# speechbrain/speechbrain

Hardware: NVIDIA H100
Metric: audio-sec/sec (RTFx) Conformer-L ASR, batch=32x10s@16kHz (higher is better)
Workload: dtype fp16 operands, fp32 accumulate/residual/softmax

## Files before the change

speechbrain_b200/csrc/encoder_ops.cu:

```cuda
#include <algorithm>

#include "common.cuh"
#include "sbk_internal.h"

namespace sbk {

constexpr int LN_MAX_PER_LANE = 32;

template <bool OUT_HALF, bool PDL, bool DUAL = false>
__global__ void __launch_bounds__(256)
layernorm_rows_kernel(const float* __restrict__ x, void* __restrict__ out, const float* __restrict__ gamma,
                      const float* __restrict__ beta, int M, int D, float eps, int act_silu,
                      __half* __restrict__ out2 = nullptr, const float* __restrict__ gamma2 = nullptr,
                      const float* __restrict__ beta2 = nullptr) {
    const int row = blockIdx.x * (blockDim.x >> 5) + (threadIdx.x >> 5);
    const int lane = threadIdx.x & 31;
    const int nv = D >> 2;
    float4 gp[PDL ? LN_MAX_PER_LANE / 4 : 1], bp[PDL ? LN_MAX_PER_LANE / 4 : 1];
    if constexpr (PDL) {
#pragma unroll
        for (int i = 0; i < LN_MAX_PER_LANE / 4; ++i) {
            const int vi = lane + i * 32;
            if (vi < nv && row < M) {
                gp[i] = __ldg(reinterpret_cast<const float4*>(gamma + vi * 4));
// ... 365 lines not shown
    const int ch = blockIdx.x * blockDim.x + threadIdx.x, b = blockIdx.y;
    if (ch >= D) return;
    float* cb = carry + static_cast<size_t>(b) * halo * D + ch;
    for (int j = 0; j < halo; ++j) {
        const int src = j + n - halo;
        cb[static_cast<size_t>(j) * D] = src >= 0 ? glu[(static_cast<size_t>(b) * n + src) * D + ch]
                                                  : (has_old ? cb[static_cast<size_t>(j + n) * D] : 0.0f);
    }
}

int dwconv_carry(const float* glu, int B, int n, int D, int K, bool has_old, float* carry, cudaStream_t stream) {
    const int halo = (K - 1) / 2;
    if (halo == 0) return SBK_OK;
    dwconv_carry_kernel<<<dim3(ceil_div(D, 128), B), 128, 0, stream>>>(glu, n, D, halo, has_old ? 1 : 0, carry);
    SBK_LAUNCH_CHECK();
    return SBK_OK;
}

void dwconv_repack_taps(const float* src, int D, int K, float* dst) {
    for (int ch = 0; ch < D; ++ch)
        for (int k = 0; k < K; ++k) dst[static_cast<size_t>(k) * D + ch] = src[static_cast<size_t>(ch) * K + k];
}

constexpr int CSGU_KMAX = CSGU_TAP_ROWS, CSGU_HALO = (CSGU_KMAX - 1) / 2;
constexpr int CSGU_TT = 64, CSGU_CC = 64, CSGU_THREADS = 256;
constexpr int CSGU_FPT = CSGU_TT / (CSGU_THREADS / CSGU_CC);
constexpr int CSGU_ROWS = CSGU_TT + CSGU_KMAX - 1;

__global__ void __launch_bounds__(256)
csgu_stats_kernel(const __half* __restrict__ u, int M, int C, float eps, float2* __restrict__ stats) {
    const int row = blockIdx.x * (blockDim.x >> 5) + (threadIdx.x >> 5);
    if (row >= M) return;
    const int lane = threadIdx.x & 31, C2 = C >> 1, nv = C2 >> 3;
    const uint4* src = reinterpret_cast<const uint4*>(u + static_cast<size_t>(row) * C + C2);
    float s = 0.0f;
    for (int j = lane; j < nv; j += 32) {
        const uint4 w = __ldg(src + j);
        const __half2* h = reinterpret_cast<const __half2*>(&w);
#pragma unroll
        for (int q = 0; q < 4; ++q) { const float2 f = __half22float2(h[q]); s += f.x + f.y; }
    }
    const float mean = warp_sum(s) / C2;
    float v = 0.0f;
    for (int j = lane; j < nv; j += 32) {
        const uint4 w = __ldg(src + j);
        const __half2* h = reinterpret_cast<const __half2*>(&w);
#pragma unroll
        for (int q = 0; q < 4; ++q) {
            const float2 f = __half22float2(h[q]);
            v += (f.x - mean) * (f.x - mean) + (f.y - mean) * (f.y - mean);
        }
    }
    const float rstd = rsqrtf(warp_sum(v) / C2 + eps);
    if (lane == 0) stats[row] = make_float2(mean, rstd);
}

__global__ void __launch_bounds__(CSGU_THREADS)
csgu_conv_gate_kernel(const __half* __restrict__ u, int T, int C, const float2* __restrict__ stats,
                      const float* __restrict__ gamma, const float* __restrict__ beta, const float* __restrict__ taps,
                      const float* __restrict__ bias, __half* __restrict__ g) {
    __shared__ __align__(16) float slab[CSGU_ROWS][CSGU_CC];
    const int C2 = C >> 1, c0 = blockIdx.x * CSGU_CC, t0 = blockIdx.y * CSGU_TT, b = blockIdx.z;
    const size_t row0 = static_cast<size_t>(b) * T;
    for (int i = threadIdx.x; i < CSGU_ROWS * (CSGU_CC / 8); i += CSGU_THREADS) {
        const int r = i / (CSGU_CC / 8), j = (i % (CSGU_CC / 8)) * 8, ch = c0 + j;
        int t = t0 - CSGU_HALO + r;
        t = t < 0 ? -t : (t >= T ? 2 * (T - 1) - t : t);
        t = min(max(t, 0), T - 1);
        float y[8] = {0.f, 0.f, 0.f, 0.f, 0.f, 0.f, 0.f, 0.f};
        if (ch < C2) {
            const float2 st = __ldg(stats + row0 + t);
            const uint4 w = __ldg(reinterpret_cast<const uint4*>(u + (row0 + t) * C + C2 + ch));
            const __half2* h = reinterpret_cast<const __half2*>(&w);
            const float4 ga = __ldg(reinterpret_cast<const float4*>(gamma + ch)), gb = __ldg(reinterpret_cast<const float4*>(gamma + ch + 4));
            const float4 ba = __ldg(reinterpret_cast<const float4*>(beta + ch)), bb = __ldg(reinterpret_cast<const float4*>(beta + ch + 4));
            const float gg[8] = {ga.x, ga.y, ga.z, ga.w, gb.x, gb.y, gb.z, gb.w};
            const float bt[8] = {ba.x, ba.y, ba.z, ba.w, bb.x, bb.y, bb.z, bb.w};
#pragma unroll
            for (int q = 0; q < 4; ++q) {
                const float2 f = __half22float2(h[q]);
                y[2 * q] = (f.x - st.x) * st.y * gg[2 * q] + bt[2 * q];
                y[2 * q + 1] = (f.y - st.x) * st.y * gg[2 * q + 1] + bt[2 * q + 1];
            }
        }
        *reinterpret_cast<float4*>(&slab[r][j]) = make_float4(y[0], y[1], y[2], y[3]);
        *reinterpret_cast<float4*>(&slab[r][j + 4]) = make_float4(y[4], y[5], y[6], y[7]);
    }
    const int cl = threadIdx.x % CSGU_CC, f0 = (threadIdx.x / CSGU_CC) * CSGU_FPT, ch = c0 + cl;
    float w[CSGU_KMAX], acc[CSGU_FPT];
    const float bz = ch < C2 ? __ldg(bias + ch) : 0.0f;
#pragma unroll
    for (int k = 0; k < CSGU_KMAX; ++k) w[k] = ch < C2 ? __ldg(taps + static_cast<size_t>(k) * C2 + ch) : 0.0f;
#pragma unroll
    for (int i = 0; i < CSGU_FPT; ++i) acc[i] = bz;
    __syncthreads();
#pragma unroll
    for (int r = 0; r < CSGU_FPT + CSGU_KMAX - 1; ++r) {
        const float xv = slab[f0 + r][cl];
#pragma unroll
        for (int i = 0; i < CSGU_FPT; ++i)
            if (r - i >= 0 && r - i < CSGU_KMAX) acc[i] = fmaf(xv, w[r - i], acc[i]);
    }
    __syncthreads();
#pragma unroll
    for (int i = 0; i < CSGU_FPT; ++i) slab[f0 + i][cl] = acc[i];
    __syncthreads();
    for (int i = threadIdx.x; i < CSGU_TT * (CSGU_CC / 8); i += CSGU_THREADS) {
        const int r = i / (CSGU_CC / 8), j = (i % (CSGU_CC / 8)) * 8, t = t0 + r;
        if (t >= T || c0 + j >= C2) continue;
        const uint4 av = __ldg(reinterpret_cast<const uint4*>(u + (row0 + t) * C + c0 + j));
        const __half2* ah = reinterpret_cast<const __half2*>(&av);
        const float4 x0 = *reinterpret_cast<const float4*>(&slab[r][j]), x1 = *reinterpret_cast<const float4*>(&slab[r][j + 4]);
        const float xs[8] = {x0.x, x0.y, x0.z, x0.w, x1.x, x1.y, x1.z, x1.w};
        uint4 o;
        uint32_t* op = reinterpret_cast<uint32_t*>(&o);
#pragma unroll
        for (int q = 0; q < 4; ++q) {
            const float2 af = __half22float2(ah[q]);
            __half2 hv = floats2half2_sat(af.x * xs[2 * q], af.y * xs[2 * q + 1]);
            op[q] = *reinterpret_cast<uint32_t*>(&hv);
        }
        *reinterpret_cast<uint4*>(g + (row0 + t) * C2 + c0 + j) = o;
    }
}

int csgu_forward(const __half* u, int B, int T, int C, const float* gamma, const float* beta, float eps, const float* taps,
                 const float* bias, int K, float2* stats, __half* g, cudaStream_t stream) {
    SBK_REQUIRE(C % 16 == 0, "csgu: csgu_linear_units=%d must be a multiple of 16 (C/2 %% 8 == 0)", C);
    SBK_REQUIRE((K & 1) == 1 && K <= CSGU_KMAX, "csgu: kernel_size=%d must be odd and <= %d", K, CSGU_KMAX);
    SBK_REQUIRE(T > (K - 1) / 2, "csgu: reflect padding needs T > (kernel_size - 1) / 2 (T=%d, kernel_size=%d)", T, K);
    SBK_REQUIRE(B <= 65535, "csgu: B=%d", B);
    SBK_REQUIRE(((reinterpret_cast<uintptr_t>(u) | reinterpret_cast<uintptr_t>(g) | reinterpret_cast<uintptr_t>(gamma) |
                  reinterpret_cast<uintptr_t>(beta)) & 15) == 0, "csgu: operands must be 16-byte aligned");
    const int M = B * T;
    if (M == 0) return SBK_OK;
    csgu_stats_kernel<<<ceil_div(M, 8), 256, 0, stream>>>(u, M, C, eps, stats);
    SBK_LAUNCH_CHECK();
    csgu_conv_gate_kernel<<<dim3(ceil_div(C / 2, CSGU_CC), ceil_div(T, CSGU_TT), B), CSGU_THREADS, 0, stream>>>(
        u, T, C, stats, gamma, beta, taps, bias, g);
    SBK_LAUNCH_CHECK();
    return SBK_OK;
}

void csgu_repack_taps(const float* src, int C2, int K, float* dst) {
    const int off = CSGU_HALO - (K - 1) / 2;
    for (size_t i = 0; i < static_cast<size_t>(CSGU_KMAX) * C2; ++i) dst[i] = 0.0f;
    for (int ch = 0; ch < C2; ++ch)
        for (int k = 0; k < K; ++k) dst[static_cast<size_t>(k + off) * C2 + ch] = src[static_cast<size_t>(ch) * K + k];
}

constexpr int ATT_BQ = 64;
constexpr int ATT_BK = 64;
constexpr int ATT_GW = 80;
constexpr int ATT_PW = ATT_BQ - 16 + ATT_GW;
constexpr int ATT_PR = ATT_PW + ATT_BK;

__device__ __forceinline__ void ldmatrix_x2_trans(uint32_t& r0, uint32_t& r1, const void* p) {
    asm volatile("ldmatrix.sync.aligned.m8n8.x2.trans.shared.b16 {%0,%1}, [%2];" : "=r"(r0), "=r"(r1) : "r"(smem_u32(p)));
}
__device__ __forceinline__ void ldmatrix_x4(uint32_t& r0, uint32_t& r1, uint32_t& r2, uint32_t& r3, const void* p) {
    asm volatile("ldmatrix.sync.aligned.m8n8.x4.shared.b16 {%0,%1,%2,%3}, [%4];"
                 : "=r"(r0), "=r"(r1), "=r"(r2), "=r"(r3) : "r"(smem_u32(p)));
}
__device__ __forceinline__ void ldmatrix_x2(uint32_t& r0, uint32_t& r1, const void* p) {
    asm volatile("ldmatrix.sync.aligned.m8n8.x2.shared.b16 {%0,%1}, [%2];" : "=r"(r0), "=r"(r1) : "r"(smem_u32(p)));
}
__device__ __forceinline__ void ldmatrix_x4_trans(uint32_t& r0, uint32_t& r1, uint32_t& r2, uint32_t& r3, const void* p) {
    asm volatile("ldmatrix.sync.aligned.m8n8.x4.trans.shared.b16 {%0,%1,%2,%3}, [%4];"
                 : "=r"(r0), "=r"(r1), "=r"(r2), "=r"(r3) : "r"(smem_u32(p)));
}
__device__ __forceinline__ float ex2_ftz(float x) {
    float y;
    asm("ex2.approx.ftz.f32 %0, %1;" : "=f"(y) : "f"(x));
    return y;
}
__device__ __forceinline__ void mma16816(float (&d)[4], const uint32_t (&a)[4], uint32_t b0, uint32_t b1) {
    asm volatile(
        "mma.sync.aligned.m16n8k16.row.col.f32.f16.f16.f32 {%0,%1,%2,%3}, {%4,%5,%6,%7}, {%8,%9}, {%0,%1,%2,%3};"
        : "+f"(d[0]), "+f"(d[1]), "+f"(d[2]), "+f"(d[3])
        : "r"(a[0]), "r"(a[1]), "r"(a[2]), "r"(a[3]), "r"(b0), "r"(b1));
}
__device__ __forceinline__ uint32_t pack_half2(float a, float b) {
    __half2 h = floats2half2_sat(a, b);
    return *reinterpret_cast<uint32_t*>(&h);
}

template <int DH, int DHP, bool RELPOS>
__host__ __device__ constexpr bool att_kv2() { return (DH % 8 == 0) && (DHP == DH) && !(RELPOS && DH == 80); }

template <int DH, int DHP, bool RELPOS, bool STREAM = false>
__global__ void __launch_bounds__(128)
encoder_attention_kernel(const __half* __restrict__ qkv, int ld, int T, const int* __restrict__ lens,
                         const float* __restrict__ pos_u, const float* __restrict__ pos_v,
                         const __half* __restrict__ P, int ldp, float scale, __half* __restrict__ out, int ldo,
                         int chunk, int left_chunks, AttStream sa) {
    constexpr int STR = DHP + 8;
    constexpr int KS = DHP / 16;
    constexpr int GW = ATT_GW;
    constexpr int VPR = DH / 4;
    extern __shared__ __align__(16) uint8_t att_smem[];
    __half* Qs = reinterpret_cast<__half*>(att_smem);
    __half* Ks = Qs + ATT_BQ * STR;
    __half* Vs = Ks + ATT_BK * STR;
    __half* Qv = Vs + ATT_BK * STR;
    __half* Ps = Qv + ATT_BQ * STR;
    float* Gs = reinterpret_cast<float*>(Ps + (RELPOS ? ATT_PR : 0) * STR);
    constexpr bool ASYNC = (DH % 8 == 0) && (DHP == DH);
    constexpr bool KV2 = att_kv2<DH, DHP, RELPOS>();
    __half* KV1 = reinterpret_cast<__half*>(Gs + (RELPOS ? 4 * 16 * (GW + 1) : 0));

    const int q_off = STREAM ? T - sa.nq : 0;
    const int b = blockIdx.z, h = blockIdx.y, i0 = q_off + blockIdx.x * ATT_BQ;
    const int warp = threadIdx.x >> 5, lane = threadIdx.x & 31, g = lane >> 2, c = lane & 3;
    const int len = lens ? min(lens[b], T) : T;
    const __half* base = STREAM ? nullptr : qkv + static_cast<size_t>(b) * T * ld + h * 3 * DH;
    auto q_row = [&](int i) {
        if constexpr (STREAM) return sa.q + (static_cast<size_t>(b) * sa.nq + (i - q_off)) * sa.ldq + h * DH;
        else return base + static_cast<size_t>(i) * ld;
    };
    auto k_row = [&](int j) {
        if constexpr (STREAM) {
            const int slot = sa.start + j < sa.cap ? sa.start + j : sa.start + j - sa.cap;
            return sa.kv + (static_cast<size_t>(b) * sa.cap + slot) * sa.ldkv + h * 2 * DH;
        } else {
            return base + static_cast<size_t>(j) * ld + DH;
        }
    };

    if constexpr (DHP != DH) {
        constexpr int PADC = DHP - DH;
        const int n_rows_pad = 4 * ATT_BQ + (RELPOS ? ATT_PR : 0);
        for (int i = threadIdx.x; i < n_rows_pad * PADC; i += blockDim.x) {
            const int r = i / PADC, cc = i - r * PADC;
            Qs[r * STR + DH + cc] = __float2half(0.0f);
        }
    }
    for (int i = threadIdx.x; i < ATT_BQ * VPR; i += blockDim.x) {
        const int r = i / VPR, v4 = i - r * VPR;
        uint2 val = make_uint2(0, 0);
        if (i0 + r < T) val = *reinterpret_cast<const uint2*>(q_row(i0 + r) + v4 * 4);
        if constexpr (RELPOS) {
            const __half* hv = reinterpret_cast<const __half*>(&val);
            __half qu[4], qv[4];
#pragma unroll
            for (int e = 0; e < 4; ++e) {
                const float q = __half2float(hv[e]);
                qu[e] = float2half_sat((q + __ldg(pos_u + h * DH + v4 * 4 + e)) * scale);
                qv[e] = float2half_sat((q + __ldg(pos_v + h * DH + v4 * 4 + e)) * scale);
            }
            *reinterpret_cast<uint2*>(Qs + r * STR + v4 * 4) = *reinterpret_cast<uint2*>(qu);
            *reinterpret_cast<uint2*>(Qv + r * STR + v4 * 4) = *reinterpret_cast<uint2*>(qv);
        } else {
            *reinterpret_cast<uint2*>(Qs + r * STR + v4 * 4) = val;
        }
    }
    __syncthreads();

    uint32_t qa[KS][4];
    uint32_t qva[RELPOS ? KS : 1][4];
    {
        const __half* q0 = Qs + (warp * 16 + g) * STR + 2 * c;
#pragma unroll
        for (int ks = 0; ks < KS; ++ks) {
            qa[ks][0] = *reinterpret_cast<const uint32_t*>(q0 + ks * 16);
            qa[ks][1] = *reinterpret_cast<const uint32_t*>(q0 + 8 * STR + ks * 16);
            qa[ks][2] = *reinterpret_cast<const uint32_t*>(q0 + ks * 16 + 8);
            qa[ks][3] = *reinterpret_cast<const uint32_t*>(q0 + 8 * STR + ks * 16 + 8);
        }
        if constexpr (RELPOS) {
            const __half* v0 = Qv + (warp * 16 + g) * STR + 2 * c;
#pragma unroll
            for (int ks = 0; ks < KS; ++ks) {
                qva[ks][0] = *reinterpret_cast<const uint32_t*>(v0 + ks * 16);
                qva[ks][1] = *reinterpret_cast<const uint32_t*>(v0 + 8 * STR + ks * 16);
                qva[ks][2] = *reinterpret_cast<const uint32_t*>(v0 + ks * 16 + 8);
                qva[ks][3] = *reinterpret_cast<const uint32_t*>(v0 + 8 * STR + ks * 16 + 8);
            }
        }
    }

    float o[DHP / 8][4];
#pragma unroll
    for (int i = 0; i < DHP / 8; ++i) o[i][0] = o[i][1] = o[i][2] = o[i][3] = 0.0f;
    float m_run[2] = {-INFINITY, -INFINITY}, l_run[2] = {0.0f, 0.0f};
    const float LOG2E = 1.4426950408889634f;
    int blk_begin = 0, n_blk = (len + ATT_BK - 1) / ATT_BK;
    int klo[2] = {0, 0}, khi[2] = {len, len};
    if (chunk > 0) {
        const int i_last = min(i0 + ATT_BQ, T) - 1;
        const int hi_last = min(len, (i_last / chunk + 1) * chunk);
        n_blk = (hi_last + ATT_BK - 1) / ATT_BK;
        if (left_chunks >= 0) blk_begin = max(0, (i0 / chunk - left_chunks) * chunk) / ATT_BK;
#pragma unroll
        for (int r = 0; r < 2; ++r) {
            const int i = min(i0 + warp * 16 + g + 8 * r, T - 1);
            khi[r] = min(len, (i / chunk + 1) * chunk);
            klo[r] = left_chunks >= 0 ? max(0, (i / chunk - left_chunks) * chunk) : 0;
        }
    }

    auto p_first = [&](int jb) { return i0 - jb * ATT_BK - (ATT_BK - 1); };
    auto p_slot = [](int v) {
        const int s = v % ATT_PR;
        return s < 0 ? s + ATT_PR : s;
    };
    auto p_src = [&](int v) { return P + static_cast<size_t>(min(v < 0 ? -v : v, T - 1)) * ldp + h * DH; };
    auto stage_async = [&](int jb, __half* kd, __half* vd) {
        const int j0 = jb * ATT_BK;
        constexpr int V8 = DH / 8;
        for (int i = threadIdx.x; i < ATT_BK * V8; i += blockDim.x) {
            const int r = i / V8, v8 = i - r * V8;
            const bool ok = j0 + r < T;
            const __half* rowp = k_row(ok ? j0 + r : 0) + v8 * 8;
            const uint32_t nbytes = ok ? 16u : 0u;
            asm volatile("cp.async.cg.shared.global [%0], [%1], 16, %2;" ::"r"(smem_u32(kd + r * STR + v8 * 8)),
                         "l"(rowp), "r"(nbytes) : "memory");
            asm volatile("cp.async.cg.shared.global [%0], [%1], 16, %2;" ::"r"(smem_u32(vd + r * STR + v8 * 8)),
                         "l"(rowp + DH), "r"(nbytes) : "memory");
        }
        if constexpr (RELPOS) {
            const int a = p_first(jb), n = jb == blk_begin ? ATT_PW : ATT_BK;
            for (int i = threadIdx.x; i < n * V8; i += blockDim.x) {
                const int x = i / V8, v8 = i - x * V8;
                asm volatile("cp.async.cg.shared.global [%0], [%1], 16;" ::"r"(smem_u32(Ps + p_slot(a + x) * STR + v8 * 8)),
                             "l"(p_src(a + x) + v8 * 8) : "memory");
            }
        }
        asm volatile("cp.async.commit_group;" ::: "memory");
    };
    auto stage_p8 = [&](int jb) {
        const int a = p_first(jb), n = jb == blk_begin ? ATT_PW : ATT_BK;
        for (int i = threadIdx.x; i < n * VPR; i += blockDim.x) {
            const int x = i / VPR, v4 = i - x * VPR;
            asm volatile("cp.async.ca.shared.global [%0], [%1], 8;" ::"r"(smem_u32(Ps + p_slot(a + x) * STR + v4 * 4)),
                         "l"(p_src(a + x) + v4 * 4) : "memory");
        }
        asm volatile("cp.async.commit_group;" ::: "memory");
    };
    if (n_blk > blk_begin) {
        if constexpr (ASYNC) stage_async(blk_begin, Ks, Vs);
        else if constexpr (RELPOS) stage_p8(blk_begin);
    }

    for (int jb = blk_begin; jb < n_blk; ++jb) {
        const int j0 = jb * ATT_BK;
        const __half* Kc = Ks;
        const __half* Vc = Vs;
        if constexpr (KV2) {
            if ((jb - blk_begin) & 1) { Kc = KV1; Vc = KV1 + ATT_BK * STR; }
            asm volatile("cp.async.wait_group 0;" ::: "memory");
            __syncthreads();
            if (jb + 1 < n_blk) {
                if ((jb - blk_begin) & 1) stage_async(jb + 1, Ks, Vs);
                else stage_async(jb + 1, KV1, KV1 + ATT_BK * STR);
            }
        } else if constexpr (ASYNC) {
            if (jb != blk_begin) {
                __syncthreads();
                stage_async(jb, Ks, Vs);
            }
            asm volatile("cp.async.wait_group 0;" ::: "memory");
            __syncthreads();
        } else {
            if constexpr (RELPOS) asm volatile("cp.async.wait_group 0;" ::: "memory");
            __syncthreads();
            if constexpr (RELPOS) {
                if (jb + 1 < n_blk) stage_p8(jb + 1);
            }
            for (int i = threadIdx.x; i < ATT_BK * VPR; i += blockDim.x) {
                const int r = i / VPR, v4 = i - r * VPR;
                uint2 kv = make_uint2(0, 0), vv = make_uint2(0, 0);
                if (j0 + r < T) {
                    const __half* rowp = k_row(j0 + r) + v4 * 4;
                    kv = *reinterpret_cast<const uint2*>(rowp);
                    vv = *reinterpret_cast<const uint2*>(rowp + DH);
                }
                *reinterpret_cast<uint2*>(Ks + r * STR + v4 * 4) = kv;
                *reinterpret_cast<uint2*>(Vs + r * STR + v4 * 4) = vv;
            }
            __syncthreads();
        }

        float s[ATT_BK / 8][4];
#pragma unroll
        for (int nt = 0; nt < ATT_BK / 8; ++nt) {
            s[nt][0] = s[nt][1] = s[nt][2] = s[nt][3] = 0.0f;
            const __half* kp = Kc + (nt * 8 + (lane & 7)) * STR + (lane >> 3) * 8;
#pragma unroll
            for (int ks = 0; ks + 1 < KS; ks += 2) {
                uint32_t b0, b1, b2, b3;
                ldmatrix_x4(b0, b1, b2, b3, kp + ks * 16);
                mma16816(s[nt], qa[ks], b0, b1);
                mma16816(s[nt], qa[ks + 1], b2, b3);
            }
            if constexpr (KS & 1) {
                uint32_t b0, b1;
                ldmatrix_x2(b0, b1, Kc + (nt * 8 + (lane & 7)) * STR + ((lane >> 3) & 1) * 8 + (KS - 1) * 16);
                mma16816(s[nt], qa[KS - 1], b0, b1);
            }
        }
        if constexpr (RELPOS) {
            float* Gw = Gs + warp * 16 * (GW + 1);
            const int rmin = p_first(jb) + warp * 16;
#pragma unroll 1
            for (int nt = 0; nt < GW / 8; ++nt) {
                float gacc[4] = {0.f, 0.f, 0.f, 0.f};
                const __half* pp = Ps + p_slot(rmin + nt * 8 + g) * STR + 2 * c;
#pragma unroll
                for (int ks = 0; ks < KS; ++ks)
                    mma16816(gacc, qva[ks], *reinterpret_cast<const uint32_t*>(pp + ks * 16),
                             *reinterpret_cast<const uint32_t*>(pp + ks * 16 + 8));
                const int col = nt * 8 + 2 * c;
                Gw[g * (GW + 1) + col] = gacc[0];
                Gw[g * (GW + 1) + col + 1] = gacc[1];
                Gw[(g + 8) * (GW + 1) + col] = gacc[2];
                Gw[(g + 8) * (GW + 1) + col + 1] = gacc[3];
            }
            __syncwarp();
#pragma unroll
            for (int nt = 0; nt < ATT_BK / 8; ++nt) {
#pragma unroll
                for (int e = 0; e < 4; ++e) {
                    const int li = g + (e >> 1) * 8, lj = nt * 8 + 2 * c + (e & 1);
                    s[nt][e] += Gw[li * (GW + 1) + (li - lj + ATT_BK - 1)];
                }
            }
            __syncwarp();
        }
        float mx[2] = {-INFINITY, -INFINITY};
        if (chunk > 0) {
#pragma unroll
            for (int nt = 0; nt < ATT_BK / 8; ++nt)
#pragma unroll
                for (int e = 0; e < 4; ++e) {
                    const int j = j0 + nt * 8 + 2 * c + (e & 1);
                    if (j < klo[e >> 1] || j >= khi[e >> 1]) s[nt][e] = -INFINITY;
                }
        } else if (j0 + ATT_BK > len) {
#pragma unroll
            for (int nt = 0; nt < ATT_BK / 8; ++nt)
#pragma unroll
                for (int e = 0; e < 4; ++e)
                    if (j0 + nt * 8 + 2 * c + (e & 1) >= len) s[nt][e] = -INFINITY;
        }
#pragma unroll
        for (int nt = 0; nt < ATT_BK / 8; ++nt)
#pragma unroll
            for (int e = 0; e < 4; ++e) mx[e >> 1] = fmaxf(mx[e >> 1], s[nt][e]);
        float alpha[2];
#pragma unroll
        for (int r = 0; r < 2; ++r) {
            mx[r] = fmaxf(mx[r], __shfl_xor_sync(0xffffffffu, mx[r], 1));
            mx[r] = fmaxf(mx[r], __shfl_xor_sync(0xffffffffu, mx[r], 2));
            const float m_new = fmaxf(m_run[r], mx[r]);
            alpha[r] = m_new == -INFINITY ? 1.0f : ex2_ftz((m_run[r] - m_new) * LOG2E);
            m_run[r] = m_new;
        }
        float rs[2] = {0.0f, 0.0f};
        uint32_t pa[ATT_BK / 16][4];
#pragma unroll
        for (int nt = 0; nt < ATT_BK / 8; ++nt) {
            const float ms0 = m_run[0] == -INFINITY ? 0.0f : m_run[0] * LOG2E, ms1 = m_run[1] == -INFINITY ? 0.0f : m_run[1] * LOG2E;
            const float p0 = ex2_ftz(fmaf(s[nt][0], LOG2E, -ms0)), p1 = ex2_ftz(fmaf(s[nt][1], LOG2E, -ms0));
            const float p2 = ex2_ftz(fmaf(s[nt][2], LOG2E, -ms1)), p3 = ex2_ftz(fmaf(s[nt][3], LOG2E, -ms1));
            rs[0] += p0 + p1;
            rs[1] += p2 + p3;
            pa[nt >> 1][(nt & 1) * 2 + 0] = pack_half2(p0, p1);
            pa[nt >> 1][(nt & 1) * 2 + 1] = pack_half2(p2, p3);
        }
#pragma unroll
        for (int r = 0; r < 2; ++r) {
            rs[r] += __shfl_xor_sync(0xffffffffu, rs[r], 1);
            rs[r] += __shfl_xor_sync(0xffffffffu, rs[r], 2);
            l_run[r] = l_run[r] * alpha[r] + rs[r];
        }
#pragma unroll
        for (int nt = 0; nt < DHP / 8; ++nt) {
            o[nt][0] *= alpha[0]; o[nt][1] *= alpha[0];
            o[nt][2] *= alpha[1]; o[nt][3] *= alpha[1];
        }
#pragma unroll
        for (int kk = 0; kk < ATT_BK / 16; ++kk) {
#pragma unroll
            for (int nt = 0; nt + 1 < DHP / 8; nt += 2) {
                uint32_t b0, b1, b2, b3;
                ldmatrix_x4_trans(b0, b1, b2, b3, Vc + (kk * 16 + (lane & 15)) * STR + nt * 8 + (lane >> 4) * 8);
                mma16816(o[nt], pa[kk], b0, b1);
                mma16816(o[nt + 1], pa[kk], b2, b3);
            }
            if constexpr ((DHP / 8) & 1) {
                uint32_t b0, b1;
                ldmatrix_x2_trans(b0, b1, Vc + (kk * 16 + (lane & 15)) * STR + (DHP / 8 - 1) * 8);
                mma16816(o[DHP / 8 - 1], pa[kk], b0, b1);
            }
        }
    }
    const int r0 = i0 + warp * 16 + g, r1 = r0 + 8;
    const float inv0 = l_run[0] > 0.0f ? 1.0f / l_run[0] : 0.0f, inv1 = l_run[1] > 0.0f ? 1.0f / l_run[1] : 0.0f;
    auto o_row = [&](int r) {
        const size_t row = STREAM ? static_cast<size_t>(b) * sa.nq + (r - q_off) : static_cast<size_t>(b) * T + r;
        return out + row * ldo + h * DH;
    };
#pragma unroll
    for (int nt = 0; nt < DHP / 8; ++nt) {
        const int col = nt * 8 + 2 * c;
        if (col >= DH) continue;
        if (r0 < T) *reinterpret_cast<uint32_t*>(o_row(r0) + col) = pack_half2(o[nt][0] * inv0, o[nt][1] * inv0);
        if (r1 < T) *reinterpret_cast<uint32_t*>(o_row(r1) + col) = pack_half2(o[nt][2] * inv1, o[nt][3] * inv1);
    }
}

template <int DH, int DHP, bool STREAM = false>
static int launch_encoder_attention(const __half* qkv, int ld, int B, int T, int H, const int* lens, bool relpos,
                                    const float* pos_u, const float* pos_v, const __half* P, int ldp, float scale,
                                    __half* out, int ldo, int chunk, int left_chunks, cudaStream_t stream,
                                    const AttStream& sa = AttStream{}) {
    constexpr int STR = DHP + 8;
    dim3 grid(ceil_div(STREAM ? sa.nq : T, ATT_BQ), H, B);
    if (!relpos) {
        const size_t smem = 4ull * ATT_BQ * STR * 2 + 2ull * ATT_BK * STR * 2;
        auto kern = encoder_attention_kernel<DH, DHP, false, STREAM>;
        SBK_CUDA_CHECK(cudaFuncSetAttribute(kern, cudaFuncAttributeMaxDynamicSharedMemorySize, (int)smem));
        kern<<<grid, 128, smem, stream>>>(qkv, ld, T, lens, nullptr, nullptr, nullptr, 0, scale, out, ldo, chunk, left_chunks, sa);
    } else if constexpr (DH > 64 && DH != 80) {
        set_error("encoder_attention: RelPosMHAXL with head_dim=%d not built", DH);
        return SBK_ERR_UNSUPPORTED;
    } else {
        constexpr bool ASYNC = (DH % 8 == 0) && (DHP == DH);
        if (ASYNC)
            SBK_REQUIRE(ldp % 8 == 0 && (reinterpret_cast<uintptr_t>(P) & 15) == 0, "encoder_attention: P must be 16-byte aligned");
        else
            SBK_REQUIRE(ldp % 4 == 0 && (reinterpret_cast<uintptr_t>(P) & 7) == 0, "encoder_attention: P must be 8-byte aligned");
        const size_t smem = (4ull * ATT_BQ + ATT_PR) * STR * 2 + 4ull * 16 * (ATT_GW + 1) * 4 +
                            (att_kv2<DH, DHP, true>() ? 2ull * ATT_BK * STR * 2 : 0);
        auto kern = encoder_attention_kernel<DH, DHP, true, STREAM>;
        SBK_CUDA_CHECK(cudaFuncSetAttribute(kern, cudaFuncAttributeMaxDynamicSharedMemorySize, (int)smem));
        kern<<<grid, 128, smem, stream>>>(qkv, ld, T, lens, pos_u, pos_v, P, ldp, scale, out, ldo, chunk, left_chunks, sa);
    }
    SBK_LAUNCH_CHECK();
    return SBK_OK;
}

int encoder_attention(const __half* qkv, int ld, int B, int T, int H, int head_dim, const int* lens, bool relpos,
                      const float* pos_u, const float* pos_v, const __half* P, int ldp, float scale, __half* out,
                      int ldo, cudaStream_t stream, int chunk, int left_chunks) {
    SBK_REQUIRE(chunk >= 0, "encoder_attention: chunk size must be >= 0");
    SBK_REQUIRE(ld % 4 == 0 && ldo % 2 == 0, "encoder_attention: bad leading dims");
    if (head_dim % 8 == 0)
        SBK_REQUIRE(ld % 8 == 0 && (reinterpret_cast<uintptr_t>(qkv) & 15) == 0, "encoder_attention: qkv must be 16-byte aligned");
    if (head_dim == 64)
        return launch_encoder_attention<64, 64>(qkv, ld, B, T, H, lens, relpos, pos_u, pos_v, P, ldp, scale, out, ldo, chunk, left_chunks, stream);
    if (head_dim == 36)
        return launch_encoder_attention<36, 48>(qkv, ld, B, T, H, lens, relpos, pos_u, pos_v, P, ldp, scale, out, ldo, chunk, left_chunks, stream);
    if (head_dim == 32)
        return launch_encoder_attention<32, 32>(qkv, ld, B, T, H, lens, relpos, pos_u, pos_v, P, ldp, scale, out, ldo, chunk, left_chunks, stream);
    if (head_dim == 80)
        return launch_encoder_attention<80, 80>(qkv, ld, B, T, H, lens, relpos, pos_u, pos_v, P, ldp, scale, out, ldo, chunk, left_chunks, stream);
    if (head_dim == 128)
        return launch_encoder_attention<128, 128>(qkv, ld, B, T, H, lens, relpos, pos_u, pos_v, P, ldp, scale, out, ldo, chunk, left_chunks, stream);
    set_error("encoder_attention: head_dim=%d not built (128, 80, 64, 36, 32)", head_dim);
    return SBK_ERR_UNSUPPORTED;
}

int encoder_attention_stream(const AttStream& sa, int B, int W, int H, int head_dim, bool relpos, const float* pos_u,
                             const float* pos_v, const __half* P, int ldp, float scale, __half* out, int ldo,
                             cudaStream_t stream) {
    SBK_REQUIRE(sa.nq >= 1 && sa.nq <= W && W <= sa.cap && sa.start >= 0 && sa.start < sa.cap,
                "encoder_attention_stream: bad window (%d queries, %d rows, ring of %d from %d)", sa.nq, W, sa.cap, sa.start);
    SBK_REQUIRE(sa.ldq % 8 == 0 && sa.ldkv % 8 == 0 && ldo % 2 == 0 && (reinterpret_cast<uintptr_t>(sa.q) & 15) == 0 &&
                    (reinterpret_cast<uintptr_t>(sa.kv) & 15) == 0,
                "encoder_attention_stream: q / kv must be 16-byte aligned");
    if (head_dim == 64)
        return launch_encoder_attention<64, 64, true>(nullptr, 0, B, W, H, nullptr, relpos, pos_u, pos_v, P, ldp, scale, out, ldo, 0, -1, stream, sa);
    if (head_dim == 36 && relpos)
        return launch_encoder_attention<36, 48, true>(nullptr, 0, B, W, H, nullptr, relpos, pos_u, pos_v, P, ldp, scale, out, ldo, 0, -1, stream, sa);
    if (head_dim == 32)
        return launch_encoder_attention<32, 32, true>(nullptr, 0, B, W, H, nullptr, relpos, pos_u, pos_v, P, ldp, scale, out, ldo, 0, -1, stream, sa);
    set_error("encoder_attention_stream: head_dim=%d not built (64, 36 with RelPosMHAXL, 32)", head_dim);
    return SBK_ERR_UNSUPPORTED;
}

__global__ void stream_qkv_kernel(const float* __restrict__ qkv, int n, int H, int DH, const float* __restrict__ inv_freq,
                                  long long pos0, float q_scale, __half* __restrict__ q, __half* __restrict__ kv, int cap,
                                  int slot0) {
    const int half_dh = DH >> 1, d = H * DH;
    const int idx = blockIdx.x * blockDim.x + threadIdx.x;
    if (idx >= H * half_dh) return;
    const int h = idx / half_dh, p = idx - h * half_dh, row = blockIdx.y, b = row / n, i = row - b * n;
    const float* src = qkv + static_cast<size_t>(row) * 3 * d + h * 3 * DH + 2 * p;
    float q0 = src[0], q1 = src[1], k0 = src[DH], k1 = src[DH + 1];
    if (inv_freq) {
        double sd, cd;
        sincos(static_cast<double>(pos0 + i) * static_cast<double>(inv_freq[p]), &sd, &cd);
        const float c = static_cast<float>(cd), s = static_cast<float>(sd);
        const float rq0 = (q0 * c - q1 * s) * q_scale, rq1 = (q1 * c + q0 * s) * q_scale;
        const float rk0 = k0 * c - k1 * s, rk1 = k1 * c + k0 * s;
        q0 = rq0; q1 = rq1; k0 = rk0; k1 = rk1;
    }
    *reinterpret_cast<__half2*>(q + static_cast<size_t>(row) * d + h * DH + 2 * p) = floats2half2_sat(q0, q1);
    const int slot = (slot0 + i) % cap;
    __half* dst = kv + (static_cast<size_t>(b) * cap + slot) * 2 * d + h * 2 * DH + 2 * p;
    *reinterpret_cast<__half2*>(dst) = floats2half2_sat(k0, k1);
    *reinterpret_cast<__half2*>(dst + DH) = floats2half2_sat(src[2 * DH], src[2 * DH + 1]);
}

int stream_qkv(const float* qkv, int B, int n, int H, int DH, const float* inv_freq, long long pos0, float q_scale,
               __half* q, __half* kv, int cap, int slot0, cudaStream_t stream) {
    SBK_REQUIRE(DH % 2 == 0 && n >= 1 && cap >= n && slot0 >= 0, "stream_qkv: bad shape");
    const int pairs = H * DH / 2;
    stream_qkv_kernel<<<dim3(ceil_div(pairs, 128), B * n), 128, 0, stream>>>(qkv, n, H, DH, inv_freq, pos0, q_scale, q, kv,
                                                                            cap, slot0);
    SBK_LAUNCH_CHECK();
    return SBK_OK;
}

constexpr int HM_WARPS = 8, HM_THREADS = 32 * HM_WARPS, HM_TILE = 64, HM_CHUNK = 256;

__device__ __forceinline__ void hm_mma_tile(float (&acc)[4], const __half* A, int lda, const __half* Bm, int ldb, int K) {
    const int lane = threadIdx.x & 31;
    const __half* pa = A + (lane & 15) * lda + (lane >> 4) * 8;
    const __half* pb = Bm + (lane & 7) * ldb + ((lane >> 3) & 1) * 8;
    for (int k0 = 0; k0 < K; k0 += 16) {
        uint32_t a[4], b0, b1;
        ldmatrix_x4(a[0], a[1], a[2], a[3], pa + k0);
        ldmatrix_x2(b0, b1, pb + k0);
        mma16816(acc, a, b0, b1);
    }
}

template <typename Epi>
__device__ __forceinline__ void hm_gemm(const __half* A, int lda, const __half* Bm, int ldb, int R, int N, int K, Epi epi) {
    const int warp = threadIdx.x >> 5, lane = threadIdx.x & 31, g = lane >> 2, c = lane & 3;
    const int nt = N / 8, tiles = (R / 16) * nt;
    for (int t = warp; t < tiles; t += HM_WARPS) {
        const int r0 = (t / nt) * 16, n0 = (t % nt) * 8;
        float acc[4] = {0.0f, 0.0f, 0.0f, 0.0f};
        hm_mma_tile(acc, A + r0 * lda, lda, Bm + n0 * ldb, ldb, K);
        epi(r0 + g, n0 + 2 * c, acc[0], acc[1]);
        epi(r0 + g + 8, n0 + 2 * c, acc[2], acc[3]);
    }
}

__device__ __forceinline__ void hm_copy_rows(__half* dst, int ld, const __half* __restrict__ src, int rows, int cols) {
    const int v = cols / 8;
    for (int i = threadIdx.x; i < rows * v; i += blockDim.x) {
        const int r = i / v, j = (i - r * v) * 8;
        *reinterpret_cast<uint4*>(dst + r * ld + j) = __ldg(reinterpret_cast<const uint4*>(src + static_cast<size_t>(r) * cols + j));
    }
}

template <int E>
__device__ __forceinline__ void hm_stage(const __half* __restrict__ h16, const float* __restrict__ pe, int d, int T, int len,
                                         size_t row0, int t0, int rows, int ch0, __half* hin, int ldh, __half* xmT, int ldx) {
    constexpr int V = E / 8;
    for (int i = threadIdx.x; i < rows * V; i += blockDim.x) {
        const int r = i / V, v = (i - r * V) * 8, t = t0 + r;
        uint4 raw = make_uint4(0u, 0u, 0u, 0u), hv = make_uint4(0u, 0u, 0u, 0u);
        if (t < len) raw = __ldg(reinterpret_cast<const uint4*>(h16 + (row0 + t) * d + ch0 + v));
        const __half* xh = reinterpret_cast<const __half*>(&raw);
        if (t < T) {
            const float4 p0 = __ldg(reinterpret_cast<const float4*>(pe + static_cast<size_t>(t) * d + ch0 + v));
            const float4 p1 = __ldg(reinterpret_cast<const float4*>(pe + static_cast<size_t>(t) * d + ch0 + v + 4));
            hv.x = pack_half2(__half2float(xh[0]) + p0.x, __half2float(xh[1]) + p0.y);
            hv.y = pack_half2(__half2float(xh[2]) + p0.z, __half2float(xh[3]) + p0.w);
            hv.z = pack_half2(__half2float(xh[4]) + p1.x, __half2float(xh[5]) + p1.y);
            hv.w = pack_half2(__half2float(xh[6]) + p1.z, __half2float(xh[7]) + p1.w);
        }
        *reinterpret_cast<uint4*>(hin + r * ldh + v) = hv;
        if (xmT != nullptr) {
#pragma unroll
            for (int j = 0; j < 8; ++j) xmT[(v + j) * ldx + r] = xh[j];
        }
    }
}

template <int E>
__global__ void __launch_bounds__(HM_THREADS)
hypermix_reduce_kernel(const __half* __restrict__ h16, int T, int d, int KH, const int* __restrict__ lens,
                       const float* __restrict__ pe, const __half* __restrict__ fc1w, const float* __restrict__ fc1b,
                       const __half* __restrict__ fc2w, const float* __restrict__ fc2b, float* __restrict__ part, int nchunk) {
    constexpr int LE = E + 8, LT = HM_TILE + 8;
    constexpr int MAXT = E / 4;
    extern __shared__ __align__(16) uint8_t hm_smem[];
    __half* w1s = reinterpret_cast<__half*>(hm_smem);
    __half* w2s = w1s + E * LE;
    __half* hin = w2s + KH * LE;
    __half* hid = hin + HM_TILE * LE;
    __half* xmT = hid + HM_TILE * LE;
    __half* w1T = xmT + E * LT;
    const int chunk = blockIdx.x, m = blockIdx.y, b = blockIdx.z, M = gridDim.y;
    const int warp = threadIdx.x >> 5, lane = threadIdx.x & 31, g = lane >> 2, c = lane & 3;
    const int len = lens ? min(max(lens[b], 0), T) : T;
    const size_t row0 = static_cast<size_t>(b) * T;
    const float* b1 = fc1b + m * E;
    const float* b2 = fc2b + m * KH;
    hm_copy_rows(w1s, LE, fc1w + static_cast<size_t>(m) * E * E, E, E);
    hm_copy_rows(w2s, LE, fc2w + static_cast<size_t>(m) * KH * E, KH, E);
    const int nt = KH / 8, tiles = (E / 16) * nt;
    float acc[MAXT][4];
#pragma unroll
    for (int i = 0; i < MAXT; ++i) acc[i][0] = acc[i][1] = acc[i][2] = acc[i][3] = 0.0f;
    const int te = min(chunk * HM_CHUNK + HM_CHUNK, len);
// ... 328 lines not shown
```

Baseline: 46500.

## Pipeline attention K/V/P loads with multi-stage mbarrier ring and shared tiles across query blocks

Restructures the encoder attention kernel into an S-stage cp.async ring buffer tracked by mbarriers, with the stage count picked from the per-SM shared memory budget. When the grid is large enough, two 64-row query tiles share one CTA, so the K/V/P tiles are loaded once for both. Q fragments now go straight from global memory into registers instead of through shared memory, and the non-async 8-byte path is folded into the same staging code. This aims to hide load latency and cut redundant K/V traffic. In exchange it brings more __syncthreads, larger CTAs and more complex range handling, which could lower occupancy.

New measurement: 47120 (median of 6 runs). 1.3% higher.

```diff
diff --git a/speechbrain_b200/csrc/encoder_ops.cu b/speechbrain_b200/csrc/encoder_ops.cu
--- a/speechbrain_b200/csrc/encoder_ops.cu
+++ b/speechbrain_b200/csrc/encoder_ops.cu
@@ -541,8 +541,6 @@
 constexpr int ATT_BQ = 64;
 constexpr int ATT_BK = 64;
 constexpr int ATT_GW = 80;
-constexpr int ATT_PW = ATT_BQ - 16 + ATT_GW;
-constexpr int ATT_PR = ATT_PW + ATT_BK;
 
 __device__ __forceinline__ void ldmatrix_x2_trans(uint32_t& r0, uint32_t& r1, const void* p) {
     asm volatile("ldmatrix.sync.aligned.m8n8.x2.trans.shared.b16 {%0,%1}, [%2];" : "=r"(r0), "=r"(r1) : "r"(smem_u32(p)));
@@ -574,33 +572,47 @@
     return *reinterpret_cast<uint32_t*>(&h);
 }
 
-template <int DH, int DHP, bool RELPOS>
-__host__ __device__ constexpr bool att_kv2() { return (DH % 8 == 0) && (DHP == DH) && !(RELPOS && DH == 80); }
+__host__ __device__ constexpr int att_pw(int nq) { return nq * ATT_BQ - 16 + ATT_GW; }
+
+template <int DHP, bool RELPOS>
+__host__ __device__ constexpr size_t att_smem_bytes(int nq, int S) {
+    constexpr size_t ROW = (DHP + 8) * sizeof(__half);
+    return (RELPOS ? 4ull * nq * 16 * (ATT_GW + 1) * sizeof(float) + (att_pw(nq) + (S - 1) * ATT_BK) * ROW : 0) +
+           2ull * S * ATT_BK * ROW + S * sizeof(uint64_t);
+}
+
+template <int n>
+__device__ __forceinline__ void att_cp_async(void* dst, const void* src, bool ok = true) {
+    if constexpr (n == 16)
+        asm volatile("cp.async.cg.shared.global [%0], [%1], 16, %2;" ::"r"(smem_u32(dst)), "l"(src), "r"(ok ? 16u : 0u)
+                     : "memory");
+    else
+        asm volatile("cp.async.ca.shared.global [%0], [%1], %2, %3;" ::"r"(smem_u32(dst)), "l"(src), "n"(n),
+                     "r"(ok ? unsigned(n) : 0u) : "memory");
+}
 
 template <int DH, int DHP, bool RELPOS, bool STREAM = false>
-__global__ void __launch_bounds__(128)
+__global__ void __launch_bounds__(2 * 128, DH <= 64 ? 2 : 1)
 encoder_attention_kernel(const __half* __restrict__ qkv, int ld, int T, const int* __restrict__ lens,
                          const float* __restrict__ pos_u, const float* __restrict__ pos_v,
                          const __half* __restrict__ P, int ldp, float scale, __half* __restrict__ out, int ldo,
-                         int chunk, int left_chunks, AttStream sa) {
+                         int chunk, int left_chunks, int S, AttStream sa) {
     constexpr int STR = DHP + 8;
     constexpr int KS = DHP / 16;
     constexpr int GW = ATT_GW;
-    constexpr int VPR = DH / 4;
+    constexpr int CP = DH % 8 == 0 ? 8 : 4;
+    constexpr int VPR = DH / CP;
+    const int nw = blockDim.x >> 5, nq = nw >> 2, PR = att_pw(nq) + (S - 1) * ATT_BK;
     extern __shared__ __align__(16) uint8_t att_smem[];
-    __half* Qs = reinterpret_cast<__half*>(att_smem);
-    __half* Ks = Qs + ATT_BQ * STR;
-    __half* Vs = Ks + ATT_BK * STR;
-    __half* Qv = Vs + ATT_BK * STR;
-    __half* Ps = Qv + ATT_BQ * STR;
-    float* Gs = reinterpret_cast<float*>(Ps + (RELPOS ? ATT_PR : 0) * STR);
-    constexpr bool ASYNC = (DH % 8 == 0) && (DHP == DH);
-    constexpr bool KV2 = att_kv2<DH, DHP, RELPOS>();
-    __half* KV1 = reinterpret_cast<__half*>(Gs + (RELPOS ? 4 * 16 * (GW + 1) : 0));
+    float* Gs = reinterpret_cast<float*>(att_smem);
+    __half* Ks = reinterpret_cast<__half*>(Gs + (RELPOS ? nw * 16 * (GW + 1) : 0));
+    __half* Vs = Ks + S * ATT_BK * STR;
+    __half* Ps = Vs + S * ATT_BK * STR;
+    uint64_t* full = reinterpret_cast<uint64_t*>(Ps + (RELPOS ? PR : 0) * STR);
 
     const int q_off = STREAM ? T - sa.nq : 0;
-    const int b = blockIdx.z, h = blockIdx.y, i0 = q_off + blockIdx.x * ATT_BQ;
-    const int warp = threadIdx.x >> 5, lane = threadIdx.x & 31, g = lane >> 2, c = lane & 3;
+    const int warp = threadIdx.x >> 5, wq = warp & 3, lane = threadIdx.x & 31, g = lane >> 2, c = lane & 3;
+    const int b = blockIdx.z, h = blockIdx.y, i0c = q_off + blockIdx.x * nq * ATT_BQ, i0 = i0c + (warp >> 2) * ATT_BQ;
     const int len = lens ? min(lens[b], T) : T;
     const __half* base = STREAM ? nullptr : qkv + static_cast<size_t>(b) * T * ld + h * 3 * DH;
     auto q_row = [&](int i) {
@@ -616,159 +628,108 @@
         }
     };
 
+    auto blk_range = [&](int q0, int& begin, int& end) {
+        begin = 0;
+        end = (len + ATT_BK - 1) / ATT_BK;
+        if (chunk > 0) {
+            const int i_last = min(q0 + ATT_BQ, T) - 1;
+            end = (min(len, (i_last / chunk + 1) * chunk) + ATT_BK - 1) / ATT_BK;
+            if (left_chunks >= 0) begin = max(0, (q0 / chunk - left_chunks) * chunk) / ATT_BK;
+        }
+    };
+    int blk_begin, n_blk;
+    blk_range(i0, blk_begin, n_blk);
+    if (i0 >= T) n_blk = 0;
+    int cb, ce;
+    {
+        int e;
+        blk_range(i0c, cb, e);
+        blk_range(min(i0c + (nq - 1) * ATT_BQ, q_off + ((T - q_off - 1) / ATT_BQ) * ATT_BQ), e, ce);
+    }
+
     if constexpr (DHP != DH) {
         constexpr int PADC = DHP - DH;
-        const int n_rows_pad = 4 * ATT_BQ + (RELPOS ? ATT_PR : 0);
+        const int n_rows_pad = 2 * S * ATT_BK + (RELPOS ? PR : 0);
         for (int i = threadIdx.x; i < n_rows_pad * PADC; i += blockDim.x) {
             const int r = i / PADC, cc = i - r * PADC;
-            Qs[r * STR + DH + cc] = __float2half(0.0f);
-        }
-    }
-    for (int i = threadIdx.x; i < ATT_BQ * VPR; i += blockDim.x) {
-        const int r = i / VPR, v4 = i - r * VPR;
-        uint2 val = make_uint2(0, 0);
-        if (i0 + r < T) val = *reinterpret_cast<const uint2*>(q_row(i0 + r) + v4 * 4);
+            Ks[r * STR + DH + cc] = __float2half(0.0f);
+        }
+    }
+    if (threadIdx.x < S) mbar_init(full + threadIdx.x, blockDim.x);
+    __syncthreads();
+
+    auto p_first = [&](int jb) { return i0c - jb * ATT_BK - (ATT_BK - 1); };
+    auto p_slot = [&](int v) {
+        const int s = v % PR;
+        return s < 0 ? s + PR : s;
+    };
+    auto p_src = [&](int v) { return P + static_cast<size_t>(min(v < 0 ? -v : v, T - 1)) * ldp + h * DH; };
+    auto stage = [&](int jb, int s) {
+        const int j0 = jb * ATT_BK;
+        __half* kd = Ks + s * ATT_BK * STR;
+        __half* vd = Vs + s * ATT_BK * STR;
+        for (int i = threadIdx.x; i < ATT_BK * VPR; i += blockDim.x) {
+            const int r = i / VPR, col = (i - r * VPR) * CP;
+            const bool ok = j0 + r < T;
+            const __half* rowp = k_row(ok ? j0 + r : 0) + col;
+            att_cp_async<2 * CP>(kd + r * STR + col, rowp, ok);
+            att_cp_async<2 * CP>(vd + r * STR + col, rowp + DH, ok);
+        }
         if constexpr (RELPOS) {
-            const __half* hv = reinterpret_cast<const __half*>(&val);
-            __half qu[4], qv[4];
-#pragma unroll
-            for (int e = 0; e < 4; ++e) {
-                const float q = __half2float(hv[e]);
-                qu[e] = float2half_sat((q + __ldg(pos_u + h * DH + v4 * 4 + e)) * scale);
-                qv[e] = float2half_sat((q + __ldg(pos_v + h * DH + v4 * 4 + e)) * scale);
-            }
-            *reinterpret_cast<uint2*>(Qs + r * STR + v4 * 4) = *reinterpret_cast<uint2*>(qu);
-            *reinterpret_cast<uint2*>(Qv + r * STR + v4 * 4) = *reinterpret_cast<uint2*>(qv);
-        } else {
-            *reinterpret_cast<uint2*>(Qs + r * STR + v4 * 4) = val;
-        }
-    }
-    __syncthreads();
+            const int a = p_first(jb), n = jb == cb ? att_pw(nq) : ATT_BK;
+            for (int i = threadIdx.x; i < n * VPR; i += blockDim.x) {
+                const int x = i / VPR, col = (i - x * VPR) * CP;
+                att_cp_async<2 * CP>(Ps + p_slot(a + x) * STR + col, p_src(a + x) + col);
+            }
+        }
+        asm volatile("cp.async.mbarrier.arrive.noinc.shared::cta.b64 [%0];" ::"r"(smem_u32(full + s)) : "memory");
+    };
+    for (int k = 0; k < S && cb + k < ce; ++k) stage(cb + k, k);
 
     uint32_t qa[KS][4];
     uint32_t qva[RELPOS ? KS : 1][4];
-    {
-        const __half* q0 = Qs + (warp * 16 + g) * STR + 2 * c;
-#pragma unroll
-        for (int ks = 0; ks < KS; ++ks) {
-            qa[ks][0] = *reinterpret_cast<const uint32_t*>(q0 + ks * 16);
-            qa[ks][1] = *reinterpret_cast<const uint32_t*>(q0 + 8 * STR + ks * 16);
-            qa[ks][2] = *reinterpret_cast<const uint32_t*>(q0 + ks * 16 + 8);
-            qa[ks][3] = *reinterpret_cast<const uint32_t*>(q0 + 8 * STR + ks * 16 + 8);
-        }
-        if constexpr (RELPOS) {
-            const __half* v0 = Qv + (warp * 16 + g) * STR + 2 * c;
-#pragma unroll
-            for (int ks = 0; ks < KS; ++ks) {
-                qva[ks][0] = *reinterpret_cast<const uint32_t*>(v0 + ks * 16);
-                qva[ks][1] = *reinterpret_cast<const uint32_t*>(v0 + 8 * STR + ks * 16);
-                qva[ks][2] = *reinterpret_cast<const uint32_t*>(v0 + ks * 16 + 8);
-                qva[ks][3] = *reinterpret_cast<const uint32_t*>(v0 + 8 * STR + ks * 16 + 8);
-            }
-        }
-    }
+#pragma unroll
+    for (int ks = 0; ks < KS; ++ks)
+#pragma unroll
+        for (int e = 0; e < 4; ++e) {
+            const int i = i0 + wq * 16 + g + (e & 1) * 8, col = ks * 16 + 2 * c + (e >> 1) * 8;
+            uint32_t w = 0, wv = 0;
+            if (col < DH) {
+                if (i < T) w = *reinterpret_cast<const uint32_t*>(q_row(i) + col);
+                if constexpr (RELPOS) {
+                    const __half* hv = reinterpret_cast<const __half*>(&w);
+                    __half qu[2], qv[2];
+#pragma unroll
+                    for (int k = 0; k < 2; ++k) {
+                        const float q = __half2float(hv[k]);
+                        qu[k] = float2half_sat((q + __ldg(pos_u + h * DH + col + k)) * scale);
+                        qv[k] = float2half_sat((q + __ldg(pos_v + h * DH + col + k)) * scale);
+                    }
+                    w = *reinterpret_cast<uint32_t*>(qu);
+                    wv = *reinterpret_cast<uint32_t*>(qv);
+                }
+            }
+            qa[ks][e] = w;
+            if constexpr (RELPOS) qva[ks][e] = wv;
+        }
 
     float o[DHP / 8][4];
 #pragma unroll
     for (int i = 0; i < DHP / 8; ++i) o[i][0] = o[i][1] = o[i][2] = o[i][3] = 0.0f;
     float m_run[2] = {-INFINITY, -INFINITY}, l_run[2] = {0.0f, 0.0f};
     const float LOG2E = 1.4426950408889634f;
-    int blk_begin = 0, n_blk = (len + ATT_BK - 1) / ATT_BK;
-    int klo[2] = {0, 0}, khi[2] = {len, len};
-    if (chunk > 0) {
-        const int i_last = min(i0 + ATT_BQ, T) - 1;
-        const int hi_last = min(len, (i_last / chunk + 1) * chunk);
-        n_blk = (hi_last + ATT_BK - 1) / ATT_BK;
-        if (left_chunks >= 0) blk_begin = max(0, (i0 / chunk - left_chunks) * chunk) / ATT_BK;
-#pragma unroll
-        for (int r = 0; r < 2; ++r) {
-            const int i = min(i0 + warp * 16 + g + 8 * r, T - 1);
-            khi[r] = min(len, (i / chunk + 1) * chunk);
-            klo[r] = left_chunks >= 0 ? max(0, (i / chunk - left_chunks) * chunk) : 0;
-        }
-    }
-
-    auto p_first = [&](int jb) { return i0 - jb * ATT_BK - (ATT_BK - 1); };
-    auto p_slot = [](int v) {
-        const int s = v % ATT_PR;
-        return s < 0 ? s + ATT_PR : s;
-    };
-    auto p_src = [&](int v) { return P + static_cast<size_t>(min(v < 0 ? -v : v, T - 1)) * ldp + h * DH; };
-    auto stage_async = [&](int jb, __half* kd, __half* vd) {
+
+    for (int jb = cb; jb < ce; ++jb) {
+        const int cur = (jb - cb) % S;
+        if (jb > cb && jb + S - 1 < ce) {
+            __syncthreads();
+            stage(jb + S - 1, cur == 0 ? S - 1 : cur - 1);
+        }
+        if (jb < blk_begin || jb >= n_blk) continue;
+        mbar_wait(full + cur, ((jb - cb) / S) & 1);
         const int j0 = jb * ATT_BK;
-        constexpr int V8 = DH / 8;
-        for (int i = threadIdx.x; i < ATT_BK * V8; i += blockDim.x) {
-            const int r = i / V8, v8 = i - r * V8;
-            const bool ok = j0 + r < T;
-            const __half* rowp = k_row(ok ? j0 + r : 0) + v8 * 8;
-            const uint32_t nbytes = ok ? 16u : 0u;
-            asm volatile("cp.async.cg.shared.global [%0], [%1], 16, %2;" ::"r"(smem_u32(kd + r * STR + v8 * 8)),
-                         "l"(rowp), "r"(nbytes) : "memory");
-            asm volatile("cp.async.cg.shared.global [%0], [%1], 16, %2;" ::"r"(smem_u32(vd + r * STR + v8 * 8)),
-                         "l"(rowp + DH), "r"(nbytes) : "memory");
-        }
-        if constexpr (RELPOS) {
-            const int a = p_first(jb), n = jb == blk_begin ? ATT_PW : ATT_BK;
-            for (int i = threadIdx.x; i < n * V8; i += blockDim.x) {
-                const int x = i / V8, v8 = i - x * V8;
-                asm volatile("cp.async.cg.shared.global [%0], [%1], 16;" ::"r"(smem_u32(Ps + p_slot(a + x) * STR + v8 * 8)),
-                             "l"(p_src(a + x) + v8 * 8) : "memory");
-            }
-        }
-        asm volatile("cp.async.commit_group;" ::: "memory");
-    };
-    auto stage_p8 = [&](int jb) {
-        const int a = p_first(jb), n = jb == blk_begin ? ATT_PW : ATT_BK;
-        for (int i = threadIdx.x; i < n * VPR; i += blockDim.x) {
-            const int x = i / VPR, v4 = i - x * VPR;
-            asm volatile("cp.async.ca.shared.global [%0], [%1], 8;" ::"r"(smem_u32(Ps + p_slot(a + x) * STR + v4 * 4)),
-                         "l"(p_src(a + x) + v4 * 4) : "memory");
-        }
-        asm volatile("cp.async.commit_group;" ::: "memory");
-    };
-    if (n_blk > blk_begin) {
-        if constexpr (ASYNC) stage_async(blk_begin, Ks, Vs);
-        else if constexpr (RELPOS) stage_p8(blk_begin);
-    }
-
-    for (int jb = blk_begin; jb < n_blk; ++jb) {
-        const int j0 = jb * ATT_BK;
-        const __half* Kc = Ks;
-        const __half* Vc = Vs;
-        if constexpr (KV2) {
-            if ((jb - blk_begin) & 1) { Kc = KV1; Vc = KV1 + ATT_BK * STR; }
-            asm volatile("cp.async.wait_group 0;" ::: "memory");
-            __syncthreads();
-            if (jb + 1 < n_blk) {
-                if ((jb - blk_begin) & 1) stage_async(jb + 1, Ks, Vs);
-                else stage_async(jb + 1, KV1, KV1 + ATT_BK * STR);
-            }
-        } else if constexpr (ASYNC) {
-            if (jb != blk_begin) {
-                __syncthreads();
-                stage_async(jb, Ks, Vs);
-            }
-            asm volatile("cp.async.wait_group 0;" ::: "memory");
-            __syncthreads();
-        } else {
-            if constexpr (RELPOS) asm volatile("cp.async.wait_group 0;" ::: "memory");
-            __syncthreads();
-            if constexpr (RELPOS) {
-                if (jb + 1 < n_blk) stage_p8(jb + 1);
-            }
-            for (int i = threadIdx.x; i < ATT_BK * VPR; i += blockDim.x) {
-                const int r = i / VPR, v4 = i - r * VPR;
-                uint2 kv = make_uint2(0, 0), vv = make_uint2(0, 0);
-                if (j0 + r < T) {
-                    const __half* rowp = k_row(j0 + r) + v4 * 4;
-                    kv = *reinterpret_cast<const uint2*>(rowp);
-                    vv = *reinterpret_cast<const uint2*>(rowp + DH);
-                }
-                *reinterpret_cast<uint2*>(Ks + r * STR + v4 * 4) = kv;
-                *reinterpret_cast<uint2*>(Vs + r * STR + v4 * 4) = vv;
-            }
-            __syncthreads();
-        }
+        const __half* Kc = Ks + cur * ATT_BK * STR;
+        const __half* Vc = Vs + cur * ATT_BK * STR;
 
         float s[ATT_BK / 8][4];
 #pragma unroll
@@ -790,11 +751,12 @@
         }
         if constexpr (RELPOS) {
             float* Gw = Gs + warp * 16 * (GW + 1);
-            const int rmin = p_first(jb) + warp * 16;
+            const int slot0 = p_slot(p_first(jb) + warp * 16 + g);
 #pragma unroll 1
             for (int nt = 0; nt < GW / 8; ++nt) {
                 float gacc[4] = {0.f, 0.f, 0.f, 0.f};
-                const __half* pp = Ps + p_slot(rmin + nt * 8 + g) * STR + 2 * c;
+                const int slot = slot0 + nt * 8 < PR ? slot0 + nt * 8 : slot0 + nt * 8 - PR;
+                const __half* pp = Ps + slot * STR + 2 * c;
 #pragma unroll
                 for (int ks = 0; ks < KS; ++ks)
                     mma16816(gacc, qva[ks], *reinterpret_cast<const uint32_t*>(pp + ks * 16),
@@ -818,6 +780,13 @@
         }
         float mx[2] = {-INFINITY, -INFINITY};
         if (chunk > 0) {
+            int klo[2], khi[2];
+#pragma unroll
+            for (int r = 0; r < 2; ++r) {
+                const int i = min(i0 + wq * 16 + g + 8 * r, T - 1);
+                khi[r] = min(len, (i / chunk + 1) * chunk);
+                klo[r] = left_chunks >= 0 ? max(0, (i / chunk - left_chunks) * chunk) : 0;
+            }
 #pragma unroll
             for (int nt = 0; nt < ATT_BK / 8; ++nt)
 #pragma unroll
@@ -884,7 +853,7 @@
             }
         }
     }
-    const int r0 = i0 + warp * 16 + g, r1 = r0 + 8;
+    const int r0 = i0 + wq * 16 + g, r1 = r0 + 8;
     const float inv0 = l_run[0] > 0.0f ? 1.0f / l_run[0] : 0.0f, inv1 = l_run[1] > 0.0f ? 1.0f / l_run[1] : 0.0f;
     auto o_row = [&](int r) {
         const size_t row = STREAM ? static_cast<size_t>(b) * sa.nq + (r - q_off) : static_cast<size_t>(b) * T + r;
@@ -904,27 +873,47 @@
                                     const float* pos_u, const float* pos_v, const __half* P, int ldp, float scale,
                                     __half* out, int ldo, int chunk, int left_chunks, cudaStream_t stream,
                                     const AttStream& sa = AttStream{}) {
-    constexpr int STR = DHP + 8;
-    dim3 grid(ceil_div(STREAM ? sa.nq : T, ATT_BQ), H, B);
-    if (!relpos) {
-        const size_t smem = 4ull * ATT_BQ * STR * 2 + 2ull * ATT_BK * STR * 2;
-        auto kern = encoder_attention_kernel<DH, DHP, false, STREAM>;
-        SBK_CUDA_CHECK(cudaFuncSetAttribute(kern, cudaFuncAttributeMaxDynamicSharedMemorySize, (int)smem));
-        kern<<<grid, 128, smem, stream>>>(qkv, ld, T, lens, nullptr, nullptr, nullptr, 0, scale, out, ldo, chunk, left_chunks, sa);
-    } else if constexpr (DH > 64 && DH != 80) {
-        set_error("encoder_attention: RelPosMHAXL with head_dim=%d not built", DH);
-        return SBK_ERR_UNSUPPORTED;
-    } else {
-        constexpr bool ASYNC = (DH % 8 == 0) && (DHP == DH);
-        if (ASYNC)
+    if constexpr (DH > 64 && DH != 80) {
+        if (relpos) {
+            set_error("encoder_attention: RelPosMHAXL with head_dim=%d not built", DH);
+            return SBK_ERR_UNSUPPORTED;
+        }
+    }
+    if (relpos) {
+        if (DH % 8 == 0)
             SBK_REQUIRE(ldp % 8 == 0 && (reinterpret_cast<uintptr_t>(P) & 15) == 0, "encoder_attention: P must be 16-byte aligned");
         else
             SBK_REQUIRE(ldp % 4 == 0 && (reinterpret_cast<uintptr_t>(P) & 7) == 0, "encoder_attention: P must be 8-byte aligned");
-        const size_t smem = (4ull * ATT_BQ + ATT_PR) * STR * 2 + 4ull * 16 * (ATT_GW + 1) * 4 +
-                            (att_kv2<DH, DHP, true>() ? 2ull * ATT_BK * STR * 2 : 0);
-        auto kern = encoder_attention_kernel<DH, DHP, true, STREAM>;
+    }
+    int dev = 0, sms = 0, smem_sm = 0, smem_rsv = 0;
+    SBK_CUDA_CHECK(cudaGetDevice(&dev));
+    SBK_CUDA_CHECK(cudaDeviceGetAttribute(&sms, cudaDevAttrMultiProcessorCount, dev));
+    SBK_CUDA_CHECK(cudaDeviceGetAttribute(&smem_sm, cudaDevAttrMaxSharedMemoryPerMultiprocessor, dev));
+    SBK_CUDA_CHECK(cudaDeviceGetAttribute(&smem_rsv, cudaDevAttrReservedSharedMemoryPerBlock, dev));
+    auto smem_bytes = [&](int nq, int S) {
+        return relpos ? att_smem_bytes<DHP, true>(nq, S) : att_smem_bytes<DHP, false>(nq, S);
+    };
+    const int nqb = ceil_div(STREAM ? sa.nq : T, ATT_BQ), nkb = ceil_div(T, ATT_BK);
+    const size_t half_sm = static_cast<size_t>(smem_sm) / 2 - smem_rsv;
+    const int nq = DH <= 64 && nqb >= 2 && static_cast<long long>(B) * H * ceil_div(nqb, 2) >= 4ll * sms &&
+                           smem_bytes(2, 2) <= half_sm ? 2 : 1;
+    const size_t budget = static_cast<size_t>(smem_sm) * nq / 4 - smem_rsv;
+    int S = 1;
+    while (S < nkb && (S < 2 || smem_bytes(nq, S + 1) <= budget)) ++S;
+    const size_t smem = smem_bytes(nq, S);
+    const dim3 grid(ceil_div(nqb, nq), H, B);
+    if (relpos) {
+        if constexpr (DH <= 64 || DH == 80) {
+            auto kern = encoder_attention_kernel<DH, DHP, true, STREAM>;
+            SBK_CUDA_CHECK(cudaFuncSetAttribute(kern, cudaFuncAttributeMaxDynamicSharedMemorySize, (int)smem));
+            kern<<<grid, 128 * nq, smem, stream>>>(qkv, ld, T, lens, pos_u, pos_v, P, ldp, scale, out, ldo, chunk,
+                                                   left_chunks, S, sa);
+        }
+    } else {
+        auto kern = encoder_attention_kernel<DH, DHP, false, STREAM>;
         SBK_CUDA_CHECK(cudaFuncSetAttribute(kern, cudaFuncAttributeMaxDynamicSharedMemorySize, (int)smem));
-        kern<<<grid, 128, smem, stream>>>(qkv, ld, T, lens, pos_u, pos_v, P, ldp, scale, out, ldo, chunk, left_chunks, sa);
+        kern<<<grid, 128 * nq, smem, stream>>>(qkv, ld, T, lens, nullptr, nullptr, nullptr, 0, scale, out, ldo, chunk,
+                                               left_chunks, S, sa);
     }
     SBK_LAUNCH_CHECK();
     return SBK_OK;
@@ -937,6 +926,8 @@
     SBK_REQUIRE(ld % 4 == 0 && ldo % 2 == 0, "encoder_attention: bad leading dims");
     if (head_dim % 8 == 0)
         SBK_REQUIRE(ld % 8 == 0 && (reinterpret_cast<uintptr_t>(qkv) & 15) == 0, "encoder_attention: qkv must be 16-byte aligned");
+    else
+        SBK_REQUIRE((reinterpret_cast<uintptr_t>(qkv) & 7) == 0, "encoder_attention: qkv must be 8-byte aligned");
     if (head_dim == 64)
         return launch_encoder_attention<64, 64>(qkv, ld, B, T, H, lens, relpos, pos_u, pos_v, P, ldp, scale, out, ldo, chunk, left_chunks, stream);
     if (head_dim == 36)
```
